# ZhangYizhao/UltraRE

Hardware: AMD Instinct MI355X
Metric: training interactions/sec + unlearn retrain wall-time, ml-1m 5-shard SISA (higher is better)
Workload: dtype f32; 1 GPU; ml1m-shaped synthetic 6040x3416, 896914 train rows, 5-shard SISA (uniform grouping), d=32, batch=30000, SGD-momentum-L2, all shards of a rank side by side; parallelism=shards x1, arch=gfx950:sramecc+:xnack-

## Files before the change

### include/ultrare_hip.h

```cpp
#ifndef ULTRARE_HIP_H
#define ULTRARE_HIP_H

#include <stdint.h>

#ifdef __cplusplus
extern "C" {
#endif

#define URE_ABI_VERSION 15
#define URE_MAX_MODELS_PER_CALL 32
#define URE_SCORE_PARTIALS 2048

int ure_abi_version(void);
const char *ure_source_hash(void);
const char *ure_last_error(void);
int ure_device_info(int dev, int *n_cu, int *wave_size, char *arch, int arch_len);

typedef struct ure_shard {
    const int32_t *ent_oid;
    const float   *ent_r;
    uint16_t      *ent_tag;
    const int32_t *ent_src;
    uint16_t      *file_tag;
    uint32_t      *inv_stage;
// ... 7 lines not shown
    float *V[2];
    float *mU;
    float *mV;
    const float *U0;
    const float *V0;
    const float *lr_host;
    int32_t lazy_rows;
    float       *snapU;
    float       *snapV;
    const float *snap_a;
    float       *snap;
    const int32_t *row_slot;
    const int32_t *perm;
    const float   *lr;
    float         *sse;
    int32_t N, n_user, n_item, d;
    int32_t batch;
    int32_t epochs;
    float   lam, mu;
    int32_t touch_mode;
    int32_t n_multi;
    const uint16_t *file_tags;
    int32_t n_split;
} ure_shard_t;

typedef struct ure_job ure_job_t;

int ure_job_create(const ure_shard_t *shards, int n_shards, ure_job_t **out);

int ure_copy_rows_batch(int32_t n, const float *const *src, float *const *dst, float *const *dst2, const int64_t *rows, int32_t k, int32_t d,
                        void *stream);

int ure_epoch_sse_batch(int32_t n, const float *const *sse, const int64_t *n_user, int32_t epochs, double *out, void *stream);
int ure_job_destroy(ure_job_t *job);
int64_t ure_job_shard_steps(const ure_job_t *job, int s);
int64_t ure_job_ticks(const ure_job_t *job);

int ure_job_train(ure_job_t *job, int64_t tick0, int64_t tick1, void *stream);
int ure_job_materialize(ure_job_t *job, int64_t ticks_done, void *stream);
int ure_job_touch_rows(ure_job_t *job, int64_t *pairs, int64_t *window_steps);
int ure_job_index_read(ure_job_t *job, int shard, int which, void *out, int64_t capacity, int64_t *bytes);
int ure_job_train_profiled(ure_job_t *job, int64_t tick0, int64_t tick1, void *stream, double *step_ms,
                           int64_t *n_step, double *assign_ms, int64_t *n_assign);

int ure_host_randperm(const int64_t *seeds, int n_perms, int64_t n, int32_t *out, int n_threads);
int ure_host_randperm_tags(const int64_t *seeds, int n_perms, int64_t n, int32_t batch, uint16_t *tags, int n_threads);
typedef struct ure_perm {
// ... 155 lines not shown
```

### ultrare_amd/_native.py

```python
import ctypes
import os

import numpy as np

_PKG = os.path.dirname(os.path.abspath(__file__))
LIB_PATH = os.path.join(_PKG, 'libultrare_hip.so')
ABI_VERSION = 15
MAX_MODELS_PER_CALL = 32

_vp = ctypes.c_void_p
_i32 = ctypes.c_int32
_i64 = ctypes.c_int64


class UreShard(ctypes.Structure):
    _fields_ = [
        ('ent_oid', _vp), ('ent_r', _vp), ('ent_tag', _vp), ('ent_src', _vp), ('file_tag', _vp), ('inv_stage', _vp), ('inv_off', _vp),
        ('sched', _vp), ('units', _vp), ('n_units', _i32), ('n_active', _i32), ('n_slots', _i64),
        ('U', _vp * 2), ('V', _vp * 2), ('mU', _vp), ('mV', _vp),
        ('U0', _vp), ('V0', _vp), ('lr_host', _vp), ('lazy_rows', _i32),
        ('snapU', _vp), ('snapV', _vp), ('snap_a', _vp), ('snap', _vp), ('row_slot', _vp),
        ('perm', _vp), ('lr', _vp), ('sse', _vp),
        ('N', _i32), ('n_user', _i32), ('n_item', _i32), ('d', _i32),
        ('batch', _i32), ('epochs', _i32),
        ('lam', ctypes.c_float), ('mu', ctypes.c_float),
        ('touch_mode', _i32), ('n_multi', _i32),
        ('file_tags', _vp), ('n_split', _i32),
    ]


class NativeError(RuntimeError):
    pass


_PROTOTYPES = {
    'ure_abi_version': (ctypes.c_int, []),
    'ure_source_hash': (ctypes.c_char_p, []),
    'ure_last_error': (ctypes.c_char_p, []),
    'ure_device_info': (ctypes.c_int, [ctypes.c_int, ctypes.POINTER(ctypes.c_int), ctypes.POINTER(ctypes.c_int),
                                       ctypes.c_char_p, ctypes.c_int]),
    'ure_job_create': (ctypes.c_int, [ctypes.POINTER(UreShard), ctypes.c_int, ctypes.POINTER(_vp)]),
    'ure_job_destroy': (ctypes.c_int, [_vp]),
    'ure_copy_rows_batch': (ctypes.c_int, [_i32, _vp, _vp, _vp, _vp, _i32, _i32, _vp]),
    'ure_epoch_sse_batch': (ctypes.c_int, [_i32, _vp, _vp, _i32, _vp, _vp]),
    'ure_job_shard_steps': (_i64, [_vp, ctypes.c_int]),
    'ure_job_ticks': (_i64, [_vp]),
    'ure_job_train': (ctypes.c_int, [_vp, _i64, _i64, _vp]),
    'ure_job_materialize': (ctypes.c_int, [_vp, _i64, _vp]),
    'ure_job_touch_rows': (ctypes.c_int, [_vp, _vp, _vp]),
    'ure_job_index_read': (ctypes.c_int, [_vp, ctypes.c_int, ctypes.c_int, _vp, _i64, ctypes.POINTER(_i64)]),
# ... 333 lines not shown
```

### ultrare_amd/csrc/mf_job.h

```cpp
#pragma once
#include <memory>

namespace ure {


static int check_descriptor(const ure_shard_t *shards, int k)
{
    const ure_shard_t &S = shards[k];
    const int n_rows = S.n_user + S.n_item;
    const bool ok = S.N > 0 && S.n_user > 0 && S.n_item > 0 && S.batch > 0 && S.epochs > 0 && pow2(S.d) && S.d >= 4 &&
                    S.d <= 256 && S.n_active >= 0 && S.n_active <= n_rows && S.units && S.n_units >= 0 &&
                    S.n_units % (kBlock / lanes_per_row(S.d)) == 0 && S.n_slots >= S.N && S.ent_oid && S.ent_r && S.ent_tag && S.ent_src &&
                    S.file_tag && S.sched && S.U[0] && S.U[1] && S.V[0] && S.V[1] && S.mU && S.mV && (S.perm || S.file_tags) && S.lr && S.sse &&
                    (!S.lazy_rows || (S.U0 && S.V0 && S.lr_host));
    if (!ok) return fail(-1, "ure_job_create: shard %d has an invalid descriptor", k);
    if (S.d != shards[0].d) return fail(-1, "ure_job_create: all shards of a job share d");
    const int steps = make_shard_aux(S).steps;
    if (steps > 65534) return fail(-1, "ure_job_create: shard %d needs %lld steps/epoch (> 65534)", k, (long long)steps);
    if (S.touch_mode && (S.n_multi < 0 || S.n_multi > S.n_active)) return fail(-1, "ure_job_create: shard %d: n_multi outside [0, n_active]", k);
    if (tag_partitioned(S.N) && !(S.inv_stage && S.inv_off)) return fail(-1, "ure_job_create: shard %d lacks inv_stage / inv_off", k);
    return 0;
}

static bool snapshot_set_ok(const ure_shard_t &S)
// ... 14 lines not shown
    if (S.touch_mode == 3 && steps > kIdxMaxSteps) return "touch_mode 3 takes at most 1008 steps per epoch (16 mask words of 63 steps)";
    if (S.touch_mode == 3 && (S.n_multi > kIdxHeavyMax || S.n_split < 0 || S.n_split > S.n_multi)) return "touch_mode 3: 0 <= n_split <= n_multi <= 256";
    if (S.touch_mode == 3 && S.batch > 200000) return "touch_mode 3 takes batches of at most 200,000 (the parts of a split row are numbered in 11 bits)";
    if (!S.lazy_rows) return "it needs lazy_rows";
    if (steps > kTouchMaxSteps) return "more than 32000 steps per epoch (the step number shares the 16-bit batch tag with the buffer bit)";
    if (S.epochs != S0.epochs || S.lam != S0.lam || S.mu != S0.mu || !std::equal(S.lr_host, S.lr_host + S.epochs, S0.lr_host)) return "the shards' optimizer schedules differ";
    return nullptr;
}

static int check_shards(const ure_shard_t *shards, int n_shards)
{
    bool touch = false;
    for (int k = 0; k < n_shards; ++k) {
        if (int rc = check_descriptor(shards, k)) return rc;
        touch = touch || shards[k].touch_mode != 0;
    }
    for (int k = 0; k < n_shards; ++k)
        if (!snapshot_set_ok(shards[k])) return fail(-1, "ure_job_create: shard %d has an incomplete snapshot set (full: snapU + snapV; compact: snap with lazy_rows; snap_a with lazy_rows)", k);
    for (int k = 0; k < n_shards && touch; ++k)
        if (const char *why = touch_refusal(shards, k, make_shard_aux(shards[k]).steps)) return fail(-1, "ure_job_create: touch mode refused for shard %d: %s", k, why);
    return 0;
}


static void plan_job(ure_job *job, const ure_shard_t *shards, int n_shards)
{
    job->host.assign(shards, shards + n_shards);
    job->d = shards[0].d;
    if (const char *e = std::getenv("URE_SHARD_FAST")) { job->shard_fast = e[0] != '0'; job->shard_sliced = e[0] == '2'; }
    if (const char *e = std::getenv("URE_INDEX_STAGED")) job->scatter_staged = e[0] != '0';
    job->ahead = shards[0].touch_mode == 2;
    job->index = shards[0].touch_mode == 3;
    for (int k = 0; k < n_shards; ++k) {
        const ure_shard_t &S = shards[k];
        const shard_aux A = make_shard_aux(S);
        const int n_rows = S.n_user + S.n_item, per_block = kBlock / lanes_per_row(S.d);
        job->aux_host.push_back(A);
        job->lr_host.emplace_back(S.lr_host ? std::vector<float>(S.lr_host, S.lr_host + S.epochs) : std::vector<float>());
        job->host[k].lr_host = nullptr;
        job->ticks = std::max(job->ticks, (int64_t)A.steps * S.epochs);
        job->row_blocks.push_back(S.touch_mode ? S.n_units / per_block + (S.n_active - S.n_multi + kBlock - 1) / kBlock
                                               : S.n_units / per_block + (S.lazy_rows ? 0 : (n_rows - S.n_active + per_block - 1) / per_block));
        job->max_n = std::max(job->max_n, S.N);
        job->max_slots = std::max(job->max_slots, S.n_slots);
        const bool small = tag_partitioned(S.N);
        (small ? job->small_shards : job->large_shards) = true;
        if (small) job->max_small_n = std::max(job->max_small_n, S.N);
        job->max_lazy = std::max<int64_t>(job->max_lazy, S.lazy_rows ? (int64_t)(n_rows - S.n_active) * (S.d / 4) : 0);
        if (S.snapU || S.snap) {
            job->snapshots = true;
            const int64_t rows = S.snap ? S.n_active : n_rows;
            job->snap_blocks = std::max<unsigned>(job->snap_blocks, (unsigned)std::max<int64_t>(1, std::min<int64_t>((rows * (S.d / 4) + kBlock - 1) / kBlock, 2048)));
        }
        job->all_file_tags = job->all_file_tags && S.file_tags != nullptr;
        if (S.touch_mode) {
            job->touch = true;
            job->index_split = job->index_split || (job->index && S.n_split > 0);
// ... 174 lines not shown
```

### ultrare_amd/csrc/mf_train.hip

```cpp
#include "tag_prep.h"

#include <algorithm>
#include <cstdlib>
#include <type_traits>
#include <vector>

#ifndef URE_KGB_NARROW
#define URE_KGB_NARROW 5
#endif
#ifndef URE_KGB_D16
#define URE_KGB_D16 5
#endif
#ifndef URE_WAVES_D16
#define URE_WAVES_D16 5
#endif
#ifndef URE_KGB_D8
#define URE_KGB_D8 5
#endif
#ifndef URE_WAVES_D8
#define URE_WAVES_D8 5
#endif
#ifndef URE_KGB_WIDE
#define URE_KGB_WIDE 4
#endif
#ifndef URE_WAVES_NARROW
#define URE_WAVES_NARROW 7
#endif
#ifndef URE_WAVES_WIDE
#define URE_WAVES_WIDE 4
#endif
#ifndef URE_TOUCH_WAVES
#define URE_TOUCH_WAVES 4
#endif
#ifndef URE_TOUCH_KGB
#define URE_TOUCH_KGB 4
#endif

namespace ure {

constexpr int kQueue = 512;
constexpr int kSegPerLane = 8;
__host__ __device__ constexpr int lanes_per_row(int d) { return d <= URE_NARROW_MAX ? d / 4 : d / 8; }

__host__ __device__ constexpr int step_kgb(int lpr, int v4) { return v4 > 1 ? URE_KGB_WIDE : lpr >= 8 ? URE_KGB_NARROW : lpr == 4 ? URE_KGB_D16 : URE_KGB_D8; }
__host__ __device__ constexpr int step_waves(int lpr, int v4) { return v4 > 1 ? URE_WAVES_WIDE : lpr >= 8 ? URE_WAVES_NARROW : lpr == 4 ? URE_WAVES_D16 : URE_WAVES_D8; }

__device__ __forceinline__ int shard_steps(const ure_shard_t &S) { return (S.N + S.batch - 1) / S.batch; }

#ifdef URE_TIMELINE
__device__ long long *g_timeline = nullptr;
#define URE_STAMP(i)                                                                                          \
    do {                                                                                                      \
        asm volatile("s_waitcnt vmcnt(0) lgkmcnt(0)" ::: "memory");                                           \
        const size_t lin_ = (size_t)blockIdx.y * gridDim.x + blockIdx.x;                                      \
        if (g_timeline && threadIdx.x == 0 && lin_ < 16384) g_timeline[((size_t)(tick & 15) * 16384 + lin_) * 8 + (i)] = wall_clock64(); \
    } while (0)
#else
#define URE_STAMP(i)
#endif

template <int LPR, int V4>
__device__ __forceinline__ void mf_step(const ure_shard_t *__restrict__ shards, const shard_aux *__restrict__ aux, int64_t tick, int shard_fast)
{
    constexpr int D = LPR * V4 * 4;
    using Row = RowVec<V4>;
    constexpr int G = kWave / LPR;
    constexpr int UPB = kBlock / LPR;
    constexpr int CAP = kSegPerLane * LPR;
    constexpr int kGB = step_kgb(LPR, V4);
    constexpr int kQueueBytes = kWavesPerBlock * kQueue * 8;
    static_assert(kTagLds <= kQueueBytes, "tag phases must fit in the queue space");
    __shared__ __attribute__((aligned(16))) char lds_raw[kQueueBytes];
    __shared__ float4 part_acc[UPB][V4][LPR];
    int (*q_oid)[kQueue] = reinterpret_cast<int (*)[kQueue]>(lds_raw);
    float (*q_r)[kQueue] = reinterpret_cast<float (*)[kQueue]>(lds_raw + kWavesPerBlock * kQueue * 4);

    int shard_idx = (int)(shard_fast ? blockIdx.x : blockIdx.y);
    int wg = (int)(shard_fast ? blockIdx.y : blockIdx.x);
    if (shard_fast >> 1) {
        const unsigned n_sh = (unsigned)shard_fast >> 8;
        const unsigned x = blockIdx.x & 7u, j = blockIdx.x >> 3;
        const unsigned jq = j / n_sh, jr = j - jq * n_sh;
        const unsigned slice = n_sh * x + jr;
        shard_idx = (int)(slice >> 3);
        wg = (int)(jq * 8 + (slice & 7u));
    }
    const ure_shard_t &S = shards[shard_idx];
    const shard_aux &A = aux[shard_idx];
    {
        const int p_epochs = S.epochs, p_nu = S.n_user, p_ni = S.n_item, p_units = S.n_units, p_act = S.n_active, p_lazy = S.lazy_rows;
        const int64_t p_slots = S.n_slots;
        const float p_lam = S.lam, p_mu = S.mu;
        asm volatile("" ::"s"(p_epochs), "s"(p_nu), "s"(p_ni), "s"(p_units), "s"(p_act), "s"(p_lazy), "s"(p_slots), "s"(p_lam), "s"(p_mu),
                     "s"(S.lr), "s"(S.sched), "s"(S.units), "s"(S.ent_oid), "s"(S.ent_r), "s"(S.ent_tag), "s"(S.U[0]), "s"(S.U[1]),
                     "s"(S.V[0]), "s"(S.V[1]), "s"(S.mU), "s"(S.mV), "s"(S.sse), "s"(A.steps), "s"(A.inv_steps), "s"(A.ride_m),
                     "s"(A.ride_ab), "s"(A.ride_c), "s"(A.ranges), "s"(A.derive_blocks));
    }
    const int steps = A.steps;
    if (tick >= (int64_t)steps * S.epochs) return;
    const int epoch = (int)epoch_of(A, tick);
    const int s = (int)(tick - (int64_t)epoch * steps);
    const int cur = (int)(tick & 1);
    const bool first = tick == 0;
    const int n_rows = S.n_user + S.n_item;
    const int wave = threadIdx.x >> 6, lane = threadIdx.x & 63;
    const int sub = lane & (LPR - 1), grp = lane / LPR;
    const float lam = S.lam, mu = S.mu, lr = ldg(S.lr + epoch);
    const int32_t *__restrict__ ent_oid = S.ent_oid;
    const float *__restrict__ ent_r = S.ent_r;
    const uint16_t *__restrict__ ent_tag = S.ent_tag + (size_t)(epoch & 1) * S.n_slots;
    int *qo = q_oid[wave];
    float *qr = q_r[wave];

    auto sgd_update = [&](const Row &wr, const Row &mr, const Row &ar, float *mom_row, float *next_row, float *snap_row) {
        Row gr, nr;
#pragma unroll
        for (int i = 0; i < V4; ++i) {
            const float4 w = wr.q[i], m4 = mr.q[i], acc = ar.q[i];
            float4 g, wn;
// ... 4 lines not shown
                g.z = __fadd_rn(__fmul_rn(mu, m4.z), g.z); g.w = __fadd_rn(__fmul_rn(mu, m4.w), g.w);
            }
            wn.x = fmaf(-lr, g.x, w.x); wn.y = fmaf(-lr, g.y, w.y);
            wn.z = fmaf(-lr, g.z, w.z); wn.w = fmaf(-lr, g.w, w.w);
            gr.q[i] = g;
            nr.q[i] = wn;
        }
        row_store<LPR, V4>(mom_row, sub, gr);
        row_store<LPR, V4>(next_row, sub, nr);
        if (snap_row) row_store<LPR, V4>(snap_row, sub, nr);
    };

    const int nbU = S.n_units / UPB;
    const int nbD = S.lazy_rows ? 0 : (n_rows - S.n_active + UPB - 1) / UPB;
    const TagRide ride = tag_ride(A, s, epoch + 1 < S.epochs);
    const int nbR = ride.count;
    const int nbRows = nbU + nbD;
    const int blk = wg;
    if (blk >= nbRows) {
        const int rb = blk - nbRows;
        if (rb >= nbR) return;
        if (ride.phase == 0) tag_partition(S, epoch + 1, ride.first + rb, lds_raw);
        else if (ride.phase == 1) tag_collect(S, ride.first + rb, lds_raw);
        else tag_derive(S, epoch + 1, ride.first + rb, A.derive_blocks);
        return;
    }
    const int local = wave * G + grp;
    const bool dense_only = blk >= nbU;
    int4 du = make_int4(-1, 0, 0, local | (1 << 16));
    if (dense_only) {
        const int idx = S.n_active + (blk - nbU) * UPB + local;
        if (idx < n_rows) du.x = ldg(S.sched + 4 * (size_t)idx);
    } else {
        du = ldg_i4(S.units + 4 * ((size_t)blk * UPB + local));
    }
    const bool have = du.x >= 0;
    const int leader = du.w & 0xFFFF, count = (du.w >> 16) & 0x3FFF;
    const bool multi = (du.w >> 30) & 1;
    const bool owner = have && local == leader;
    const bool is_user = du.x < S.n_user;
    const int row = is_user ? du.x : du.x - S.n_user;
    const size_t row_off = (size_t)(have ? row : 0) * D;
    Row w = row_zero<V4>(), m4 = w, acc = w;
    if (have) {
        w = row_load<LPR, V4>((is_user ? S.U[cur] : S.V[cur]) + row_off, sub);
    }
    if (owner && !first) m4 = row_load<LPR, V4>((is_user ? S.mU : S.mV) + row_off, sub);
    const bool snap_here = S.snap != nullptr && S.row_slot != nullptr && s == steps - 1;
    int snap_slot = -1;
    if (snap_here && owner) snap_slot = ldg(S.row_slot + du.x);
    float sse = 0.f;
    URE_STAMP(2);
    if (!dense_only) {
        const float *__restrict__ other = is_user ? S.V[cur] : S.U[cur];
        int *gq = qo + grp * CAP;
        float *gr = qr + grp * CAP;
        const int beg = du.y, end = have ? du.z : 0;
        for (int seg = beg;; seg += CAP) {
            if (!__any(seg < end)) break;
            const int p0 = seg + sub * kSegPerLane;
            const bool valid = p0 < end;
            uint4 t4 = make_uint4(0xFFFFFFFFu, 0xFFFFFFFFu, 0xFFFFFFFFu, 0xFFFFFFFFu);
            int4 o0 = make_int4(0, 0, 0, 0), o1 = o0;
            float4 r0 = make_float4(0.f, 0.f, 0.f, 0.f), r1 = r0;
            if (valid) {
                t4 = ldg_u4(ent_tag + p0);
                o0 = ldg_i4(ent_oid + p0);
                o1 = ldg_i4(ent_oid + p0 + 4);
                r0 = ldg_f4(ent_r + p0);
                r1 = ldg_f4(ent_r + p0 + 4);
            }
            const unsigned tw[4] = {t4.x, t4.y, t4.z, t4.w};
            const int ov[8] = {o0.x, o0.y, o0.z, o0.w, o1.x, o1.y, o1.z, o1.w};
            const float rv[8] = {r0.x, r0.y, r0.z, r0.w, r1.x, r1.y, r1.z, r1.w};
            unsigned mb = 0;
#pragma unroll
            for (int k = 0; k < 8; ++k) {
                const unsigned tg = (tw[k >> 1] >> ((k & 1) * 16)) & 0xFFFFu;
                mb |= (tg == (unsigned)s ? 1u : 0u) << k;
            }
            const int c = __popc(mb);
            const int inc = group_scan<LPR>(c, sub);
            const int qn = (int)group_sum<LPR>((float)c);
            int mpos = inc - c, upos = qn + sub * kSegPerLane - mpos;
#pragma unroll
            for (int k = 0; k < 8; ++k) {
                const bool hit = (mb >> k) & 1u;
                const int pos = ((hit ? mpos : upos) + grp) & (CAP - 1);
                gq[pos] = ov[k];
                gr[pos] = rv[k];
                mpos += hit ? 1 : 0;
                upos += hit ? 0 : 1;
            }
            __builtin_amdgcn_wave_barrier();
            if (seg == beg) URE_STAMP(3);
            for (int t0 = 0; __any(t0 < qn); t0 += kGB) {
                int o[kGB];
                float r[kGB];
                bool act[kGB];
                Row v[kGB];
#pragma unroll
                for (int k = 0; k < kGB; ++k) {
                    const int qi = (min(t0 + k, CAP - 1) + grp) & (CAP - 1);
                    act[k] = t0 + k < qn;
                    o[k] = gq[qi];
                    r[k] = gr[qi];
                }
#pragma unroll
                for (int k = 0; k < kGB; ++k) v[k] = row_load<LPR, V4>(other + (size_t)(act[k] ? o[k] : 0) * D, sub);
#pragma unroll
                for (int k = 0; k < kGB; ++k) {
                    const float p = group_sum<LPR>(row_dot<V4>(w, v[k]));
                    const float e = p - r[k];
                    const float ge = act[k] ? 2.0f * e : 0.0f;
                    if (act[k]) sse = fmaf(e, e, sse);
                    row_axpy<V4>(acc, ge, v[k]);
                }
            }
            __builtin_amdgcn_wave_barrier();
        }
        URE_STAMP(4);
        if (multi) {
            if (have && count > 1) {
#pragma unroll
                for (int i = 0; i < V4; ++i) part_acc[local][i][sub] = acc.q[i];
                if (sub == 0) qr[grp * CAP] = sse;
            }
            __syncthreads();
            if (owner && count > 1) {
#pragma unroll
                for (int i = 0; i < V4; ++i) {
                    float4 a4 = part_acc[leader][i][sub];
                    for (int k = 1; k < count; ++k) {
                        const float4 t = part_acc[leader + k][i][sub];
                        a4.x += t.x; a4.y += t.y; a4.z += t.z; a4.w += t.w;
                    }
                    acc.q[i] = a4;
                }
                sse = 0.f;
                for (int k = 0; k < count; ++k) sse += q_r[(leader + k) / G][((leader + k) % G) * CAP];
// ... 562 lines not shown
```

### ultrare_amd/csrc/tag_prep.h

```cpp
#pragma once
#include "ure_internal.h"

namespace ure {

constexpr int kRange = 2048;
constexpr int kMaxRanges = 1024;
constexpr int kRangeBits = 11;
static_assert((1 << kRangeBits) == kRange, "range size");

__host__ __device__ inline int tag_ranges(int n) { return (n + kRange - 1) / kRange; }
__host__ __device__ inline bool tag_partitioned(int n) { return tag_ranges(n) <= kMaxRanges; }

constexpr int kTagLdsA = (kMaxRanges + 1) * 4 + kRange * 4 + kBlock * 4;
constexpr int kTagLdsB = kRange * 2 + 2 * kMaxRanges * 4;
constexpr int kTagLds = kTagLdsA > kTagLdsB ? kTagLdsA : kTagLdsB;

struct BatchOf {
    unsigned long long M;
    __device__ explicit BatchOf(int batch) : M((0x4000000000000000ull + (unsigned long long)batch - 1) / (unsigned long long)batch) {}
    __device__ __forceinline__ int operator()(int b) const { return (int)__umul64hi((unsigned long long)b << 2, M); }
};

__device__ inline void tag_partition(const ure_shard_t &S, int epoch, int c, char *lds)
{
// ... 104 lines not shown
    const unsigned jq = j / per;
    const unsigned slice = n_sh * x + jq;
    return WgMap{(int)(slice >> 3), (int)((j - jq * per) * 8u + (slice & 7u))};
}

__device__ inline void tag_derive(const ure_shard_t &S, int epoch, int blk, int n_blk)
{
    const int32_t *__restrict__ ent_src = S.ent_src;
    const uint16_t *__restrict__ file_tag = S.file_tags ? S.file_tags + (size_t)epoch * S.N : S.file_tag;
    uint16_t *__restrict__ ent_tag = S.ent_tag + tag_buffer(S, epoch);
    const int64_t n8 = S.n_slots / 8;
    for (int64_t q = (int64_t)blk * kBlock + threadIdx.x; q < n8; q += (int64_t)n_blk * kBlock) {
        const int4 s0 = ldg_i4(ent_src + q * 8);
        const int4 s1 = ldg_i4(ent_src + q * 8 + 4);
        const int sv[8] = {s0.x, s0.y, s0.z, s0.w, s1.x, s1.y, s1.z, s1.w};
        unsigned tg[8];
#pragma unroll
        for (int k = 0; k < 8; ++k) tg[k] = sv[k] >= 0 ? (unsigned)ldg(file_tag + sv[k]) : 0xFFFFu;
        stg_u4(ent_tag + q * 8, make_uint4(tg[0] | (tg[1] << 16), tg[2] | (tg[3] << 16), tg[4] | (tg[5] << 16), tg[6] | (tg[7] << 16)));
    }
}

__host__ __device__ inline int tag_derive_blocks(int64_t n_slots) { return (int)((n_slots / 8 + kBlock - 1) / kBlock); }

struct shard_aux {
    uint64_t inv_steps;
    int32_t steps;
    int32_t ride_m;
    int32_t ride_ab;
    int32_t ride_c;
    int32_t ride_only_c;
    int32_t ranges;
    int32_t derive_blocks;
    int32_t windows;
    unsigned long long *mask[2];
    const float4 *ptab;
    unsigned long long *unit_mask;
    unsigned long long *unit_own;
    unsigned long long *pass_mask;
    unsigned long long *ahead_masks[2];
    uint8_t *unit_nf, *sched_nf;
    int32_t n_um, n_sm;
    unsigned long long *sched_mask;
    int32_t ptab_stride;
    int32_t idx_words;
    int32_t idx_chunks;
// ... 23 lines not shown
};

constexpr int kTouchWindow = 64;
constexpr int kTouchWindowBits = 6;
__host__ __device__ inline int64_t touch_last_window(const shard_aux &a, int64_t epoch) { return (epoch + 1) * a.windows - 1; }

__host__ __device__ inline bool tag_short_riders(const ure_shard_t &S)
{
    const int64_t steps = ((int64_t)S.N + S.batch - 1) / S.batch;
    return steps < 3 && S.file_tags != nullptr && S.touch_mode != 3;
}
__host__ __device__ inline bool tag_riders(const ure_shard_t &S)
{
    const int64_t steps = ((int64_t)S.N + S.batch - 1) / S.batch;
    return ((steps >= 3 && tag_partitioned(S.N)) || tag_short_riders(S)) && S.touch_mode != 3;
}

inline shard_aux make_shard_aux(const ure_shard_t &S)
{
    shard_aux a{};
    a.steps = (int32_t)(((int64_t)S.N + S.batch - 1) / S.batch);
    a.inv_steps = a.steps == 1 ? 0 : ~0ull / (uint64_t)a.steps + 1;
    a.ranges = tag_ranges(S.N);
    a.derive_blocks = tag_derive_blocks(S.n_slots);
    a.windows = (a.steps + kTouchWindow - 1) / kTouchWindow;
    a.ride_m = a.steps >= 3 && tag_partitioned(S.N) && S.touch_mode != 3 ? a.steps / 3 : 0;
    if (a.ride_m) {
        a.ride_ab = (a.ranges + a.ride_m - 1) / a.ride_m;
        a.ride_c = (a.derive_blocks + a.ride_m - 1) / a.ride_m;
    } else if (tag_short_riders(S)) {
        a.ride_only_c = 1;
        a.ride_c = (a.derive_blocks + a.steps - 1) / a.steps;
    }
    return a;
}

__host__ __device__ inline int64_t epoch_of(const shard_aux &a, int64_t tick)
{
#ifdef __HIP_DEVICE_COMPILE__
    return a.inv_steps ? (int64_t)__umul64hi((uint64_t)tick, a.inv_steps) : tick;
#else
    return tick / a.steps;
#endif
}

struct TagRide {
    int phase;
// ... 26 lines not shown
```

### ultrare_amd/csrc/tag_prep.hip

```cpp
#include "tag_prep.h"

namespace ure {

__device__ __forceinline__ int standalone_epoch(const ure_shard_t &S, int64_t tick, int pass)
{
    const int steps = (S.N + S.batch - 1) / S.batch;
    if (tick >= (int64_t)steps * S.epochs || tick % steps != 0) return -1;
    const bool riders = tag_riders(S);
    const int epoch = (int)(tick / steps);
    if (S.touch_mode == 2) {
        if (pass == 0) return tick == 0 ? 0 : -1;
        return (tick == 0 || !riders) && epoch + 1 < S.epochs ? epoch + 1 : -1;
    }
    if (pass != 0) return -1;
    if (tick != 0 && riders) return -1;
    return epoch;
}

__global__ __launch_bounds__(kBlock) void tag_partition_kernel(const ure_shard_t *__restrict__ shards, int64_t tick, int pass)
{
    __shared__ __attribute__((aligned(16))) char lds[kTagLds];
    const ure_shard_t &S = shards[blockIdx.y];
    const int epoch = standalone_epoch(S, tick, pass);
    if (epoch < 0 || !tag_partitioned(S.N) || (int)blockIdx.x >= tag_ranges(S.N)) return;
// ... 9 lines not shown
    tag_collect(S, (int)blockIdx.x, lds);
}

__global__ __launch_bounds__(kBlock) void tag_scatter_kernel(const ure_shard_t *__restrict__ shards, int64_t tick, int pass)
{
    const ure_shard_t &S = shards[blockIdx.y];
    const int epoch = standalone_epoch(S, tick, pass);
    if (epoch < 0 || tag_partitioned(S.N) || S.file_tags) return;
    const int n = S.N;
    const int32_t *__restrict__ perm = S.perm + (size_t)epoch * n;
    uint16_t *__restrict__ file_tag = S.file_tag;
    const BatchOf batch_of(S.batch);
    for (int b = blockIdx.x * kBlock + threadIdx.x; b < n; b += gridDim.x * kBlock) {
        const int j = ldg(perm + b);
        if ((unsigned)j < (unsigned)n) stg(file_tag + j, (uint16_t)batch_of(b));
    }
}

__global__ __launch_bounds__(kBlock) void tag_derive_kernel(const ure_shard_t *__restrict__ shards, int64_t tick, int pass)
{
    const ure_shard_t &S = shards[blockIdx.y];
    const int epoch = standalone_epoch(S, tick, pass);
    if (epoch < 0) return;
    tag_derive(S, epoch, (int)blockIdx.x, (int)gridDim.x);
}

int tag_prep_needed(const ure_job *job, int64_t tick)
{
    int need = 0;
    for (const ure_shard_t &S : job->host) {
        const int64_t steps = ((int64_t)S.N + S.batch - 1) / S.batch;
        if (tick >= steps * S.epochs || tick % steps != 0) continue;
        const bool riders = tag_riders(S);
        if (S.touch_mode == 2) {
            if (tick == 0) need |= 1;
            if ((tick == 0 || !riders) && tick / steps + 1 < S.epochs) need |= 2;
        } else if (tick == 0 || !riders) need |= 1;
    }
    return need;
}

void launch_tag_prep(const ure_job *job, int64_t tick, hipStream_t st, int pass)
{
    const unsigned n_shards = (unsigned)job->host.size();
    if (job->small_shards && !job->all_file_tags) {
        const unsigned ranges = (unsigned)tag_ranges(job->max_small_n);
        hipLaunchKernelGGL(tag_partition_kernel, dim3(ranges, n_shards), dim3(kBlock), 0, st, job->dev, tick, pass);
// ... 12 lines not shown
```

### ultrare_amd/engine.py

```python
import contextlib
import ctypes
import os

import numpy as np
import torch

from . import _native as nv

SCORE_PARTIALS = 2048
SERIES_SCRATCH_BYTES = 256 << 20
LAZY_ROWS = os.environ.get('URE_LAZY_ROWS', '1') != '0'
TOUCH_MAX_STEPS = 32000
TOUCH_ROW_PASSES = 2
TOUCH_UNIT_PASSES = 8
TOUCH_AHEAD_MAX_STEPS = 63
INDEX_MAX_STEPS = 1008
INDEX_HEAVY_SLOTS = 16
INDEX_SPLIT_SLOTS = 384
INDEX_HEAVY_MAX = 256
INDEX_SHORT_EPOCH_MAX_D = 64
TOUCH_MIN_TABLE_BYTES = 256 << 20


HOST_TRACE = [] if os.environ.get('URE_HOST_TRACE', '0') == '1' else None
# ... 302 lines not shown
        self._n, self._make, self._got = n, weakref.WeakMethod(make), {}

    def __len__(self):
        return self._n

    def __getitem__(self, s):
        s = s + self._n if s < 0 else s
        if not 0 <= s < self._n:
            raise IndexError(s)
        if s not in self._got:
            make = self._make()
            if make is None:
                raise ReferenceError('the job of these views is gone')
            self._got[s] = make(s)
        return self._got[s]

    def __iter__(self):
        return (self[s] for s in range(self._n))


class TrainJob:

    def __init__(self, shards, inits, perms, k, batch, epochs, lr, lam, momentum, lr_decay=1.0, lr_step=50, lazy_rows=None, snapshots=False,
                 touch=None, final_only=False, epoch_reads=False):
        assert len(shards) == len(inits) == len(perms) and len(shards) > 0
        self.shards, self.k, self.d = shards, int(k), pad_dim(int(k))
        self.batch, self.epochs = int(batch), int(epochs)
        dev = shards[0].device
        self.device = dev
        lr_host = np.array([lr * (lr_decay ** (t // lr_step)) for t in range(self.epochs)], dtype=np.float32)
        self._lr_host = lr_host
        self.lazy_rows = LAZY_ROWS if lazy_rows is None else bool(lazy_rows)
        self._fresh = 0
        steps_all = [(sh.N + self.batch - 1) // self.batch for sh in shards]
        by_rule = False
        if touch is None:
            env = os.environ.get('URE_TOUCH', 'auto')
            live = sum(sh.n_active for sh in shards) * self.d * 12
            by_rule = env == 'auto' and live > TOUCH_MIN_TABLE_BYTES and (final_only or epoch_reads)
            touch = (env == '1') or by_rule
        self.touch = bool(touch) and self.lazy_rows and max(steps_all) <= TOUCH_MAX_STEPS
        force_index = touch == 'index' or os.environ.get('URE_TOUCH_INDEX', '1') == '2' or (by_rule and self.d <= INDEX_SHORT_EPOCH_MAX_D and
                                                                                             os.environ.get('URE_TOUCH_INDEX', '1') != '0')
        self.ahead = (self.touch and bool(final_only) and max(steps_all) <= TOUCH_AHEAD_MAX_STEPS and snapshots in (False, None, 'compact')
                      and os.environ.get('URE_TOUCH_AHEAD', '1') != '0' and not force_index)
        self.index = (self.touch and not self.ahead and max(steps_all) <= INDEX_MAX_STEPS and self.batch <= 200000 and
                      (force_index or (max(steps_all) > TOUCH_AHEAD_MAX_STEPS and os.environ.get('URE_TOUCH_INDEX', '1') != '0')))
# ... 5 lines not shown
        self._arrivals = []
        self.wait_marks = None
        descs = (nv.UreShard * len(shards))()
        from . import rng
        mark('job: start')
        cur = torch.cuda.current_stream(dev) if torch.device(dev).type == 'cuda' else None
        seen = set()
        for sh in shards:
            if sh.ready is not None and id(sh.ready) not in seen:
                seen.add(id(sh.ready))
                cur.wait_event(sh.ready)
        al = lambda x: (x + 63) // 64 * 64
        d = self.d
        sizes = [(2 * sh.n_user * d, 2 * sh.n_item * d, sh.n_user * d, sh.n_item * d, self.epochs * sh.n_user,
                  sh.n_user * d if self.lazy_rows else 0, sh.n_item * d if self.lazy_rows else 0) for sh in shards]
        pool = torch.zeros(sum(al(x) for sz in sizes for x in sz), dtype=torch.float32, device=dev)
        snap_rows = [(sh.n_active if self.snapshots == 'compact' else sh.n_user + sh.n_item) if self.snapshots else 0 for sh in shards]
        snap_pool = torch.empty(sum(al(self.epochs * r * d) for r in snap_rows), dtype=torch.float32, device=dev) if self.snapshots else None
        self._pool, self._snap_pool, self._small = pool, snap_pool, small
        base, snap_base = pool.data_ptr(), (snap_pool.data_ptr() if snap_pool is not None else 0)
        at = snap_at = 0
        mark('job: pools')
        self._offs, self._snap_offs, self._perms, self._init_src = [], [], [], []
        copies = []
        for s, (sh, (U0, V0), perm) in enumerate(zip(shards, inits, perms)):
            srcs = []
            for t, n_rows in ((U0, sh.n_user), (V0, sh.n_item)):
                ev = getattr(t, '_ure_event', None)
                if ev is not None and id(ev) not in seen:
                    seen.add(id(ev))
                    cur.wait_event(ev)
                if ev is not None:
                    t.record_stream(cur)
                t = torch.as_tensor(t, dtype=torch.float32)
                assert t.shape == (n_rows, self.k)
                if t.device != torch.device(dev) or not t.is_contiguous():
                    t = t.to(dev, non_blocking=True).contiguous()
                srcs.append(t)
            self._init_src.append(srcs)
            off = []
            for x in sizes[s]:
                off.append(at)
                at += al(x)
            self._offs.append(off)
            pU, pV, pmU, pmV, psse, pU0, pV0 = (base + 4 * o for o in off)
            arrival = rng.Arrival.of(perm)
# ... 4 lines not shown
            perm = torch.as_tensor(perm)
            assert perm.shape == (self.epochs, sh.N), f'perm of shard {s} must be [epochs, N]'
            as_tags = perm.dtype == torch.int16
            perm = perm.to(device=dev, dtype=torch.int16 if as_tags else torch.int32).contiguous()
            self._perms.append(perm)
            D = descs[s]
            for name in ('ent_oid', 'ent_r', 'ent_tag', 'ent_src', 'file_tag', 'inv_stage', 'inv_off', 'sched'):
                setattr(D, name, sh.ptr(name))
            if self.index:
                nnz, st_s = sh._sched_head[:min(sh.n_active, INDEX_HEAVY_MAX), 3], steps_all[s]
                D.n_multi = int(np.count_nonzero(nnz >= INDEX_HEAVY_SLOTS * st_s))
                D.n_split = min(D.n_multi, int(np.count_nonzero(nnz >= INDEX_SPLIT_SLOTS * st_s)))
                units, n_units = sh.ptr('sched'), 0
            elif self.touch:
                long_epochs = max(steps_all) > 64
                units, n_units, n_multi = sh.units(self.d, touch=True, min_passes=TOUCH_ROW_PASSES if long_epochs else 1,
                                                   unit_passes=TOUCH_UNIT_PASSES if long_epochs else 1)
                D.n_multi = n_multi
                units = nv.ptr(units)
            else:
                units = sh.units(self.d)
                n_units = units.shape[0]
                units = nv.ptr(units)
            D.units, D.n_units, D.n_active, D.n_slots = units, n_units, sh.n_active, sh.n_slots
            D.U[0], D.U[1] = pU, pU + 4 * sh.n_user * d
            D.V[0], D.V[1] = pV, pV + 4 * sh.n_item * d
            D.mU, D.mV = pmU, pmV
            D.perm, D.lr, D.sse = (None if as_tags else nv.ptr(perm)), nv.ptr(self.lr), psse
            D.file_tags = nv.ptr(perm) if as_tags else None
            D.N, D.n_user, D.n_item, D.d = sh.N, sh.n_user, sh.n_item, self.d
            D.batch, D.epochs = self.batch, self.epochs
            D.lam, D.mu = float(lam), float(momentum)
            D.touch_mode = (3 if self.index else 2 if self.ahead else 1) if self.touch else 0
            self._snap_offs.append(snap_at)
            if self.snapshots:
                D.snap_a = small[1 + s].data_ptr()
                if self.snapshots == 'compact':
                    D.snap, D.row_slot = snap_base + 4 * snap_at, sh.ptr('_row_slot')
                else:
                    D.snapU, D.snapV = snap_base + 4 * snap_at, snap_base + 4 * (snap_at + self.epochs * sh.n_user * d)
                snap_at += al(self.epochs * snap_rows[s] * d)
            if self.lazy_rows:
                D.U0, D.V0, D.lr_host, D.lazy_rows = pU0, pV0, lr_host.ctypes.data, 1
            copies += [(srcs[0].data_ptr(), sh.n_user, pU, pU0 if self.lazy_rows else 0), (srcs[1].data_ptr(), sh.n_item, pV, pV0 if self.lazy_rows else 0)]
        n_c = len(copies)
        src_a, dst_a, dst2_a = (ctypes.c_void_p * n_c)(*[c[0] for c in copies]), (ctypes.c_void_p * n_c)(*[c[2] for c in copies]), \
# ... 137 lines not shown
        n = ctypes.c_int64()
        nv.check(nv.lib().ure_job_index_read(self._job, s, which, None, 0, ctypes.byref(n)), 'ure_job_index_read')
        out = np.empty(n.value // np.dtype(dtype).itemsize, dtype=dtype)
        nv.check(nv.lib().ure_job_index_read(self._job, s, which, out.ctypes.data, out.nbytes, ctypes.byref(n)), 'ure_job_index_read')
        return out.reshape(-1, cols) if cols > 1 else out

    def epoch_sse(self, s):
        return self.epoch_sse_queue([s]).cpu().numpy()[0]

    def epoch_sse_queue(self, which=None, out=None, stream=None):
        which = list(range(len(self.shards))) if which is None else list(which)
        n = len(which)
        out = torch.empty(n, self.epochs, dtype=torch.float64, device=self.device) if out is None else out
        assert out.shape == (n, self.epochs) and out.dtype == torch.float64 and out.is_contiguous()
        base = self._pool.data_ptr()
        ptrs = (ctypes.c_void_p * n)(*[base + 4 * self._offs[s][4] for s in which])
        rows = (ctypes.c_int64 * n)(*[self.shards[s].n_user for s in which])
        nv.check(nv.lib().ure_epoch_sse_batch(n, ptrs, rows, self.epochs, out.data_ptr(), nv.stream_handle(stream)), 'ure_epoch_sse_batch')
        return out

    def epoch_sse_all(self):
        return self.epoch_sse_queue().cpu().numpy()

    def check_tags(self):
        seen = set()
        for a in self._arrivals:
            a.check(seen)

    def close(self):
        if self._job:
            nv.lib().ure_job_destroy(self._job)
            self._job = ctypes.c_void_p()
            try:
                self.check_tags()
            finally:
                self._pool = self._snap_pool = self._small = None
                self._perms, self._arrivals = [], []
                if isinstance(getattr(self, 'state', None), _States):
                    self.state._got.clear()

    def __del__(self):
        try:
            self.close()
        except Exception:
            pass


_LOG2_TAB = np.log2(np.arange(2, 11)).astype(np.float64)
_IDCG = 1.0 + np.sum(np.ones(9) / _LOG2_TAB)
_LOG2_TAB = np.concatenate([_LOG2_TAB, [_IDCG]])


class FixedBase:

    def __init__(self, n, base):
        self.n, self.base = int(n), base

    def __len__(self):
        return self.n

# ... 707 lines not shown
```

Before: 7.714 billion interactions/s.

## Pre-sort per-unit entries into per-step runs during tag derivation

During tag derivation for the next epoch, each unit's (other-id, rating) pairs are regrouped by step tag into a contiguous run buffer, and per-step run end offsets are recorded. The training step then reads only its own run directly instead of scanning every entry of the unit and filtering by tag through the LDS queue. The aim is to remove the redundant per-step scan over all of a unit's entries. The cost is extra memory (double-buffered pair arrays and run-end tables) and a heavier derive pass. It only applies when an epoch has at most 16 steps and touch mode is off.

Measured after the change: 5.786 billion interactions/s. 25.0% lower.

```diff
diff --git a/include/ultrare_hip.h b/include/ultrare_hip.h
--- a/include/ultrare_hip.h
+++ b/include/ultrare_hip.h
@@ -53,7 +53,11 @@
     int32_t n_multi;
     const uint16_t *file_tags;
     int32_t n_split;
+    uint32_t *run_pair;
+    uint16_t *run_end;
 } ure_shard_t;
+
+#define URE_RUN_STEPS 16
 
 typedef struct ure_job ure_job_t;
 
diff --git a/ultrare_amd/_native.py b/ultrare_amd/_native.py
--- a/ultrare_amd/_native.py
+++ b/ultrare_amd/_native.py
@@ -7,6 +7,7 @@
 LIB_PATH = os.path.join(_PKG, 'libultrare_hip.so')
 ABI_VERSION = 15
 MAX_MODELS_PER_CALL = 32
+RUN_STEPS = 16
 
 _vp = ctypes.c_void_p
 _i32 = ctypes.c_int32
@@ -26,6 +27,7 @@
         ('lam', ctypes.c_float), ('mu', ctypes.c_float),
         ('touch_mode', _i32), ('n_multi', _i32),
         ('file_tags', _vp), ('n_split', _i32),
+        ('run_pair', _vp), ('run_end', _vp),
     ]
 
 
diff --git a/ultrare_amd/csrc/mf_job.h b/ultrare_amd/csrc/mf_job.h
--- a/ultrare_amd/csrc/mf_job.h
+++ b/ultrare_amd/csrc/mf_job.h
@@ -60,6 +60,11 @@
     return 0;
 }
 
+static bool runs_apply(const ure_shard_t &S)
+{
+    return S.run_pair && S.run_end && !S.touch_mode && make_shard_aux(S).steps <= kRunSteps && S.n_units > 0 && S.n_slots < ((int64_t)1 << 28);
+}
+
 
 static void plan_job(ure_job *job, const ure_shard_t *shards, int n_shards)
 {
@@ -70,7 +75,11 @@
     job->ahead = shards[0].touch_mode == 2;
     job->index = shards[0].touch_mode == 3;
     for (int k = 0; k < n_shards; ++k) {
-        const ure_shard_t &S = shards[k];
+        if (!runs_apply(shards[k])) {
+            job->host[k].run_pair = nullptr;
+            job->host[k].run_end = nullptr;
+        }
+        const ure_shard_t &S = job->host[k];
         const shard_aux A = make_shard_aux(S);
         const int n_rows = S.n_user + S.n_item, per_block = kBlock / lanes_per_row(S.d);
         job->aux_host.push_back(A);
diff --git a/ultrare_amd/csrc/mf_train.hip b/ultrare_amd/csrc/mf_train.hip
--- a/ultrare_amd/csrc/mf_train.hip
+++ b/ultrare_amd/csrc/mf_train.hip
@@ -40,7 +40,6 @@
 
 constexpr int kQueue = 512;
 constexpr int kSegPerLane = 8;
-__host__ __device__ constexpr int lanes_per_row(int d) { return d <= URE_NARROW_MAX ? d / 4 : d / 8; }
 
 __host__ __device__ constexpr int step_kgb(int lpr, int v4) { return v4 > 1 ? URE_KGB_WIDE : lpr >= 8 ? URE_KGB_NARROW : lpr == 4 ? URE_KGB_D16 : URE_KGB_D8; }
 __host__ __device__ constexpr int step_waves(int lpr, int v4) { return v4 > 1 ? URE_WAVES_WIDE : lpr >= 8 ? URE_WAVES_NARROW : lpr == 4 ? URE_WAVES_D16 : URE_WAVES_D8; }
@@ -69,7 +68,7 @@
     constexpr int CAP = kSegPerLane * LPR;
     constexpr int kGB = step_kgb(LPR, V4);
     constexpr int kQueueBytes = kWavesPerBlock * kQueue * 8;
-    static_assert(kTagLds <= kQueueBytes, "tag phases must fit in the queue space");
+    static_assert(kTagLds <= kQueueBytes && kRunLds <= kQueueBytes, "tag phases must fit in the queue space");
     __shared__ __attribute__((aligned(16))) char lds_raw[kQueueBytes];
     __shared__ float4 part_acc[UPB][V4][LPR];
     int (*q_oid)[kQueue] = reinterpret_cast<int (*)[kQueue]>(lds_raw);
@@ -94,7 +93,7 @@
         asm volatile("" ::"s"(p_epochs), "s"(p_nu), "s"(p_ni), "s"(p_units), "s"(p_act), "s"(p_lazy), "s"(p_slots), "s"(p_lam), "s"(p_mu),
                      "s"(S.lr), "s"(S.sched), "s"(S.units), "s"(S.ent_oid), "s"(S.ent_r), "s"(S.ent_tag), "s"(S.U[0]), "s"(S.U[1]),
                      "s"(S.V[0]), "s"(S.V[1]), "s"(S.mU), "s"(S.mV), "s"(S.sse), "s"(A.steps), "s"(A.inv_steps), "s"(A.ride_m),
-                     "s"(A.ride_ab), "s"(A.ride_c), "s"(A.ranges), "s"(A.derive_blocks));
+                     "s"(A.ride_ab), "s"(A.ride_c), "s"(A.ranges), "s"(A.derive_blocks), "s"(S.run_end));
     }
     const int steps = A.steps;
     if (tick >= (int64_t)steps * S.epochs) return;
@@ -145,6 +144,7 @@
         if (rb >= nbR) return;
         if (ride.phase == 0) tag_partition(S, epoch + 1, ride.first + rb, lds_raw);
         else if (ride.phase == 1) tag_collect(S, ride.first + rb, lds_raw);
+        else if (S.run_end) tag_derive_runs<LPR>(S, epoch + 1, steps, ride.first + rb, lds_raw);
         else tag_derive(S, epoch + 1, ride.first + rb, A.derive_blocks);
         return;
     }
@@ -156,6 +156,13 @@
         if (idx < n_rows) du.x = ldg(S.sched + 4 * (size_t)idx);
     } else {
         du = ldg_i4(S.units + 4 * ((size_t)blk * UPB + local));
+    }
+    const bool runs = S.run_end != nullptr;
+    int run_lo = 0, run_hi = 0;
+    if (runs && !dense_only) {
+        const uint16_t *__restrict__ re = S.run_end + ((size_t)(epoch & 1) * S.n_units + (size_t)blk * UPB + local) * kRunSteps + s;
+        run_hi = (int)ldg(re);
+        if (s > 0) run_lo = (int)ldg(re - 1);
     }
     const bool have = du.x >= 0;
     const int leader = du.w & 0xFFFF, count = (du.w >> 16) & 0x3FFF;
@@ -179,10 +186,43 @@
         int *gq = qo + grp * CAP;
         float *gr = qr + grp * CAP;
         const int beg = du.y, end = have ? du.z : 0;
+        auto train_rows = [&](const int (&o)[kGB], const float (&r)[kGB], const bool (&act)[kGB]) {
+            Row v[kGB];
+#pragma unroll
+            for (int k = 0; k < kGB; ++k) v[k] = row_load<LPR, V4>(other + (size_t)(act[k] ? o[k] : 0) * D, sub);
+#pragma unroll
+            for (int k = 0; k < kGB; ++k) {
+                const float p = group_sum<LPR>(row_dot<V4>(w, v[k]));
+                const float e = p - r[k];
+                const float ge = act[k] ? 2.0f * e : 0.0f;
+                if (act[k]) sse = fmaf(e, e, sse);
+                row_axpy<V4>(acc, ge, v[k]);
+            }
+        };
+        if (runs) {
+            const int len = end - beg;
+            const int hi = min(run_hi, len), lo = min(run_lo, hi);
+            const char *__restrict__ pr = reinterpret_cast<const char *>(S.run_pair) + (size_t)(epoch & 1) * S.n_slots * 8;
+            const int spare = hi > lo ? hi - 1 : max(min(lo, len - 1), 0);
+            for (int t0 = lo; __any(t0 < hi); t0 += kGB) {
+                int o[kGB];
+                float r[kGB];
+                bool act[kGB];
+#pragma unroll
+                for (int k = 0; k < kGB; ++k) {
+                    act[k] = t0 + k < hi;
+                    const ure_u2 p = *(const ure_u2 URE_AS1 *)(pr + (uint32_t)(beg + (act[k] ? t0 + k : spare)) * 8u);
+                    o[k] = (int)p.x;
+                    r[k] = __uint_as_float(p.y);
+                }
+                train_rows(o, r, act);
+            }
+        }
+        const int scan_end = runs ? 0 : end;
         for (int seg = beg;; seg += CAP) {
-            if (!__any(seg < end)) break;
+            if (!__any(seg < scan_end)) break;
             const int p0 = seg + sub * kSegPerLane;
-            const bool valid = p0 < end;
+            const bool valid = p0 < scan_end;
             uint4 t4 = make_uint4(0xFFFFFFFFu, 0xFFFFFFFFu, 0xFFFFFFFFu, 0xFFFFFFFFu);
             int4 o0 = make_int4(0, 0, 0, 0), o1 = o0;
             float4 r0 = make_float4(0.f, 0.f, 0.f, 0.f), r1 = r0;
@@ -221,7 +261,6 @@
                 int o[kGB];
                 float r[kGB];
                 bool act[kGB];
-                Row v[kGB];
 #pragma unroll
                 for (int k = 0; k < kGB; ++k) {
                     const int qi = (min(t0 + k, CAP - 1) + grp) & (CAP - 1);
@@ -229,16 +268,7 @@
                     o[k] = gq[qi];
                     r[k] = gr[qi];
                 }
-#pragma unroll
-                for (int k = 0; k < kGB; ++k) v[k] = row_load<LPR, V4>(other + (size_t)(act[k] ? o[k] : 0) * D, sub);
-#pragma unroll
-                for (int k = 0; k < kGB; ++k) {
-                    const float p = group_sum<LPR>(row_dot<V4>(w, v[k]));
-                    const float e = p - r[k];
-                    const float ge = act[k] ? 2.0f * e : 0.0f;
-                    if (act[k]) sse = fmaf(e, e, sse);
-                    row_axpy<V4>(acc, ge, v[k]);
-                }
+                train_rows(o, r, act);
             }
             __builtin_amdgcn_wave_barrier();
         }
diff --git a/ultrare_amd/csrc/tag_prep.h b/ultrare_amd/csrc/tag_prep.h
--- a/ultrare_amd/csrc/tag_prep.h
+++ b/ultrare_amd/csrc/tag_prep.h
@@ -150,6 +150,111 @@
 }
 
 __host__ __device__ inline int tag_derive_blocks(int64_t n_slots) { return (int)((n_slots / 8 + kBlock - 1) / kBlock); }
+
+__host__ __device__ constexpr int lanes_per_row(int d) { return d <= URE_NARROW_MAX ? d / 4 : d / 8; }
+
+constexpr int kRunSteps = URE_RUN_STEPS;
+constexpr int kRunLds = kBlock * 8 * 8;
+
+template <int LPR>
+__device__ inline void tag_derive_runs(const ure_shard_t &S, int epoch, int steps, int b, char *lds)
+{
+    constexpr int UPB = kBlock / LPR, CAP = 8 * LPR, G = kWave / LPR;
+    const int32_t *__restrict__ ent_src = S.ent_src;
+    const uint16_t *__restrict__ file_tag = S.file_tags ? S.file_tags + (size_t)epoch * S.N : S.file_tag;
+    const size_t par = (size_t)(epoch & 1);
+    uint16_t *ent_tag = S.ent_tag + par * (size_t)S.n_slots;
+    ure_u2 *pair = reinterpret_cast<ure_u2 *>(S.run_pair) + par * (size_t)S.n_slots;
+    uint16_t *run_end = S.run_end + par * (size_t)S.n_units * kRunSteps;
+    const int lane = threadIdx.x & (kWave - 1), sub = lane & (LPR - 1);
+    const int local = (threadIdx.x >> 6) * G + lane / LPR;
+    ure_u2 *stage = reinterpret_cast<ure_u2 *>(lds) + local * CAP;
+    {
+        const size_t unit = (size_t)b * UPB + local;
+        const int4 du = ldg_i4(S.units + 4 * unit);
+        const int beg = du.y, end = du.x >= 0 ? du.z : beg;
+        const bool single = end - beg <= CAP;
+        uint4 t4 = make_uint4(0xFFFFFFFFu, 0xFFFFFFFFu, 0xFFFFFFFFu, 0xFFFFFFFFu);
+        int4 o0 = make_int4(0, 0, 0, 0), o1 = o0;
+        float4 r0 = make_float4(0.f, 0.f, 0.f, 0.f), r1 = r0;
+        for (int seg = beg; seg < end; seg += CAP) {
+            const int p0 = seg + sub * 8;
+            if (p0 >= end) continue;
+            const int4 s0 = ldg_i4(ent_src + p0);
+            const int4 s1 = ldg_i4(ent_src + p0 + 4);
+            const int sv[8] = {s0.x, s0.y, s0.z, s0.w, s1.x, s1.y, s1.z, s1.w};
+            unsigned tg[8];
+#pragma unroll
+            for (int k = 0; k < 8; ++k) tg[k] = sv[k] >= 0 ? (unsigned)ldg(file_tag + sv[k]) : 0xFFFFu;
+            t4 = make_uint4(tg[0] | (tg[1] << 16), tg[2] | (tg[3] << 16), tg[4] | (tg[5] << 16), tg[6] | (tg[7] << 16));
+            stg_u4(ent_tag + p0, t4);
+        }
+        auto fetch = [&](int seg, bool tags) {
+            const int p0 = seg + sub * 8;
+            if (tags) t4 = make_uint4(0xFFFFFFFFu, 0xFFFFFFFFu, 0xFFFFFFFFu, 0xFFFFFFFFu);
+            if (p0 >= end) return false;
+            if (tags) t4 = ldg_u4(ent_tag + p0);
+            o0 = ldg_i4(S.ent_oid + p0);
+            o1 = ldg_i4(S.ent_oid + p0 + 4);
+            r0 = ldg_f4(S.ent_r + p0);
+            r1 = ldg_f4(S.ent_r + p0 + 4);
+            return true;
+        };
+        bool valid = single && fetch(beg, false);
+        unsigned e2[kRunSteps / 2];
+#pragma unroll
+        for (int j = 0; j < kRunSteps / 2; ++j) e2[j] = 0u;
+        int base = 0;
+        for (int t = 0; t <= kRunSteps; ++t) {
+            const bool rest = t == kRunSteps;
+            for (int seg = beg; seg < end && (t < steps || rest); seg += CAP) {
+                if (!single) valid = fetch(seg, true);
+                const unsigned tw[4] = {t4.x, t4.y, t4.z, t4.w};
+                const int ov[8] = {o0.x, o0.y, o0.z, o0.w, o1.x, o1.y, o1.z, o1.w};
+                const float rv[8] = {r0.x, r0.y, r0.z, r0.w, r1.x, r1.y, r1.z, r1.w};
+                unsigned mb = 0;
+#pragma unroll
+                for (int k = 0; k < 8; ++k) {
+                    const unsigned tg = (tw[k >> 1] >> ((k & 1) * 16)) & 0xFFFFu;
+                    mb |= ((rest ? tg >= (unsigned)steps : tg == (unsigned)t) ? 1u : 0u) << k;
+                }
+                if (!valid) mb = 0;
+                const int c = __popc(mb);
+                const int inc = group_scan<LPR>(c, sub);
+                const int qn = (int)group_sum<LPR>((float)c);
+                int pos = base + inc - c;
+#pragma unroll
+                for (int k = 0; k < 8; ++k) {
+                    if ((mb >> k) & 1u) {
+                        ure_u2 pr;
+                        pr.x = (unsigned)ov[k];
+                        pr.y = __float_as_uint(rv[k]);
+                        if (single) stage[pos] = pr;
+                        else *(ure_u2 URE_AS1 *)(pair + beg + pos) = pr;
+                        ++pos;
+                    }
+                }
+                base += qn;
+            }
+            if (!rest) {
+#pragma unroll
+                for (int j = 0; j + 1 < kRunSteps / 2; ++j) e2[j] = (e2[j] >> 16) | (e2[j + 1] << 16);
+                e2[kRunSteps / 2 - 1] = (e2[kRunSteps / 2 - 1] >> 16) | ((unsigned)base << 16);
+            }
+        }
+        if (sub == 0) {
+            static_assert(kRunSteps == 16, "run_end: two 16-byte stores per unit");
+            stg_u4(run_end + unit * kRunSteps, make_uint4(e2[0], e2[1], e2[2], e2[3]));
+            stg_u4(run_end + unit * kRunSteps + 8, make_uint4(e2[4], e2[5], e2[6], e2[7]));
+        }
+        __builtin_amdgcn_wave_barrier();
+        if (single) {
+            const int n2 = (end - beg) >> 1;
+            for (int i = sub; i < n2; i += LPR) *(ure_u4 URE_AS1 *)(pair + beg + 2 * i) = *reinterpret_cast<const ure_u4 *>(stage + 2 * i);
+        }
+        __builtin_amdgcn_wave_barrier();
+    }
+}
 
 struct shard_aux {
     uint64_t inv_steps;
@@ -219,7 +324,7 @@
     a.steps = (int32_t)(((int64_t)S.N + S.batch - 1) / S.batch);
     a.inv_steps = a.steps == 1 ? 0 : ~0ull / (uint64_t)a.steps + 1;
     a.ranges = tag_ranges(S.N);
-    a.derive_blocks = tag_derive_blocks(S.n_slots);
+    a.derive_blocks = S.run_pair ? S.n_units / (kBlock / lanes_per_row(S.d)) : tag_derive_blocks(S.n_slots);
     a.windows = (a.steps + kTouchWindow - 1) / kTouchWindow;
     a.ride_m = a.steps >= 3 && tag_partitioned(S.N) && S.touch_mode != 3 ? a.steps / 3 : 0;
     if (a.ride_m) {
diff --git a/ultrare_amd/csrc/tag_prep.hip b/ultrare_amd/csrc/tag_prep.hip
--- a/ultrare_amd/csrc/tag_prep.hip
+++ b/ultrare_amd/csrc/tag_prep.hip
@@ -55,7 +55,23 @@
     const ure_shard_t &S = shards[blockIdx.y];
     const int epoch = standalone_epoch(S, tick, pass);
     if (epoch < 0) return;
-    tag_derive(S, epoch, (int)blockIdx.x, (int)gridDim.x);
+    if (!S.run_pair) {
+        tag_derive(S, epoch, (int)blockIdx.x, (int)gridDim.x);
+        return;
+    }
+    __shared__ __attribute__((aligned(16))) char lds[kRunLds];
+    const int steps = (S.N + S.batch - 1) / S.batch;
+    const int lpr = lanes_per_row(S.d), n_blk = S.n_units / (kBlock / lpr);
+    for (int b = (int)blockIdx.x; b < n_blk; b += (int)gridDim.x) {
+        switch (lpr) {
+            case 1: tag_derive_runs<1>(S, epoch, steps, b, lds); break;
+            case 2: tag_derive_runs<2>(S, epoch, steps, b, lds); break;
+            case 4: tag_derive_runs<4>(S, epoch, steps, b, lds); break;
+            case 8: tag_derive_runs<8>(S, epoch, steps, b, lds); break;
+            case 16: tag_derive_runs<16>(S, epoch, steps, b, lds); break;
+            default: tag_derive_runs<32>(S, epoch, steps, b, lds); break;
+        }
+    }
 }
 
 int tag_prep_needed(const ure_job *job, int64_t tick)
diff --git a/ultrare_amd/engine.py b/ultrare_amd/engine.py
--- a/ultrare_amd/engine.py
+++ b/ultrare_amd/engine.py
@@ -348,7 +348,7 @@
 class TrainJob:
 
     def __init__(self, shards, inits, perms, k, batch, epochs, lr, lam, momentum, lr_decay=1.0, lr_step=50, lazy_rows=None, snapshots=False,
-                 touch=None, final_only=False, epoch_reads=False):
+                 touch=None, final_only=False, epoch_reads=False, sorted_runs=None):
         assert len(shards) == len(inits) == len(perms) and len(shards) > 0
         self.shards, self.k, self.d = shards, int(k), pad_dim(int(k))
         self.batch, self.epochs = int(batch), int(epochs)
@@ -400,6 +400,7 @@
         at = snap_at = 0
         mark('job: pools')
         self._offs, self._snap_offs, self._perms, self._init_src = [], [], [], []
+        self._runs = {}
         copies = []
         for s, (sh, (U0, V0), perm) in enumerate(zip(shards, inits, perms)):
             srcs = []
@@ -450,6 +451,11 @@
                 units = sh.units(self.d)
                 n_units = units.shape[0]
                 units = nv.ptr(units)
+                if sorted_runs is not False and steps_all[s] <= nv.RUN_STEPS and sh.max_row + 8 <= 0xFFFF and 0 < sh.n_slots < 1 << 28 and n_units > 0:
+                    pair_b = 2 * sh.n_slots * 8
+                    run = torch.empty(pair_b + 2 * n_units * nv.RUN_STEPS * 2, dtype=torch.uint8, device=dev)
+                    self._runs[s] = run
+                    D.run_pair, D.run_end = run.data_ptr(), run.data_ptr() + pair_b
             D.units, D.n_units, D.n_active, D.n_slots = units, n_units, sh.n_active, sh.n_slots
             D.U[0], D.U[1] = pU, pU + 4 * sh.n_user * d
             D.V[0], D.V[1] = pV, pV + 4 * sh.n_item * d
@@ -633,6 +639,13 @@
     def epoch_sse_all(self):
         return self.epoch_sse_queue().cpu().numpy()
 
+    def sorted_runs(self, s):
+        run = self._runs.get(s)
+        if run is None:
+            return None
+        pair_b = 2 * self.shards[s].n_slots * 8
+        return run[:pair_b].view(torch.int32).view(2, -1, 2), run[pair_b:].view(torch.int16).view(2, -1, nv.RUN_STEPS)
+
     def check_tags(self):
         seen = set()
         for a in self._arrivals:
@@ -646,7 +659,7 @@
                 self.check_tags()
             finally:
                 self._pool = self._snap_pool = self._small = None
-                self._perms, self._arrivals = [], []
+                self._perms, self._arrivals, self._runs = [], [], {}
                 if isinstance(getattr(self, 'state', None), _States):
                     self.state._got.clear()
 
```
